# PaddlePaddle/PASSL

Measured on AMD Instinct MI355X. Metric: images/sec/node (2-view), MoCo-v2 R50 bs256/GPU, higher is better.
Workload: dtype bf16; 1 GPU; MoCo-v2 ResNet-50 bf16, bs=256/GPU, 2x224^2 synthetic views, queue=65536, dim=128, T=0.2, m=0.999, momentum-SGD (BASELINE configs[1]); global_batch=256, parallelism=dp1, allocator_retries=0

## Files before the change

include/passl_hip.h:

```cpp
#ifndef PASSL_HIP_H_
#define PASSL_HIP_H_

#include <stdint.h>

#ifdef __cplusplus
extern "C" {
#endif

typedef void* passl_stream_t;

enum passl_status {
  PASSL_OK = 0,
  PASSL_EINVAL = -1,
  PASSL_ELAUNCH = -2,
  PASSL_EUNSUPPORTED = -3
};

enum passl_dtype { PASSL_F32 = 0, PASSL_BF16 = 1 };

#define PASSL_HIP_ABI_VERSION 16
int passl_hip_abi_version(void);
int passl_hip_set_option(const char* name, int value);
int passl_hip_get_option(const char* name, int* value);
int passl_hip_last_igemm_kernel(void);
// ... 105 lines not shown
  int64_t a_sn, a_sh, a_sw;
  int64_t dy_ld;
  float* ws;
  int64_t ws_floats;
  int32_t dtype;
  int32_t splits;
} passl_wgrad_desc;

int passl_hip_slab_reduce(const float* ws, float* out, int64_t n, int slabs, int accumulate,
                          passl_stream_t stream);
int passl_hip_conv_wgrad(const passl_wgrad_desc* d, passl_stream_t stream);


int64_t passl_hip_bn_partial_floats(int nblocks, int C, int shifted);
int passl_hip_bn_stats(const void* x, float* partial, int64_t M, int C, int nblocks, int dtype,
                       passl_stream_t stream);
int passl_hip_bn_finalize(const float* partial, int nblocks, int64_t M, int C, int rows_per_block,
                          const float* gamma, const float* beta, float* running_mean, float* running_var,
                          float momentum, float eps, float* mean, float* invstd, float* scale,
                          float* shift, passl_stream_t stream);
int passl_hip_bn_apply(const void* x, const float* scale, const float* shift, const void* residual,
                       void* z, uint8_t* relu_mask, int64_t M, int C, int relu, int dtype,
                       passl_stream_t stream);
int passl_hip_bn_bwd_reduce(const void* dz, const void* z, const void* x, const float* mean,
                            const float* invstd, const float* scale, const float* shift,
                            float* partial, int64_t M, int C, int nblocks, int relu, int dtype,
                            passl_stream_t stream);
int passl_hip_bn_bwd_finalize(const float* partial, int nblocks, int64_t M, int C,
                              const float* gamma, const float* mean, const float* invstd,
                              float* dgamma, float* dbeta, float* coef ,
                              passl_stream_t stream);
int passl_hip_bn_moments(const float* partial, int nblocks, int64_t M, int C, int rows_per_block, double* mom,
                         passl_stream_t stream);
int passl_hip_bn_finalize_moments(const double* mom_all, int world, int C, const float* gamma, const float* beta,
                                  float* running_mean, float* running_var, float momentum, float eps, float* mean,
                                  float* invstd, float* scale, float* shift, passl_stream_t stream);
int passl_hip_bn_bwd_sums(const float* partial, int nblocks, int64_t M, int C, double* sums, passl_stream_t stream);
int passl_hip_bn_bwd_finalize_sums(const double* sums_all, int world, int rank, int64_t M_total, int C,
                                   const float* gamma, const float* mean, const float* invstd, float* dgamma,
                                   float* dbeta, float* coef, passl_stream_t stream);
int passl_hip_bn_bwd_apply(const void* dz, const void* z, const void* x, const float* coef,
                           const float* scale, const float* shift, void* dx, void* dres, int64_t M,
                           int C, int relu, int dtype, passl_stream_t stream);

int passl_hip_maxpool3x3s2_fwd(const void* x, void* y, uint8_t* idx, int N, int H, int W, int C,
                               int dtype, passl_stream_t stream);
// ... 223 lines not shown
```

passl_amd/csrc/bn.hip:

```cpp
#include <mutex>
#include "common.h"
#include "bn_chunk.h"
#include "options.h"

namespace {

constexpr int kThreads = 256;


template <typename T>
__device__ __forceinline__ void apply_relu_mask(float (&g)[8], const float (&xv)[8], int relu,
                                                const void* zsrc, int64_t chunk,
                                                const float* sc, const float* sh) {
  if (relu == 1) {
    float zz[8];
    ElemTraits<T>::load8(reinterpret_cast<const T*>(zsrc) + chunk * 8, zz);
#pragma unroll
    for (int e = 0; e < 8; ++e) g[e] = zz[e] > 0.f ? g[e] : 0.f;
  } else if (relu == 2) {
#pragma unroll
    for (int e = 0; e < 8; ++e) g[e] = (xv[e] * sc[e] + sh[e]) > 0.f ? g[e] : 0.f;
  } else if (relu == 3) {
    const uint32_t bits = reinterpret_cast<const uint8_t*>(zsrc)[chunk];
#pragma unroll
// ... 342 lines not shown

__global__ void __launch_bounds__(256) bn_bwd_finalize_sums_kernel(
    const double* __restrict__ sums_all, int world, int rank, double m_total, int C,
    const float* __restrict__ gamma, const float* __restrict__ mean, const float* __restrict__ invstd,
    float* __restrict__ dgamma, float* __restrict__ dbeta, float* __restrict__ coef) {
  const int c = blockIdx.x * 256 + threadIdx.x;
  if (c >= C) return;
  double sg = 0.0, sgx = 0.0;
  for (int r = 0; r < world; ++r) {
    sg += sums_all[(int64_t)r * 2 * C + c];
    sgx += sums_all[(int64_t)r * 2 * C + C + c];
  }
  dbeta[c] += (float)sums_all[(int64_t)rank * 2 * C + c];
  dgamma[c] += (float)sums_all[(int64_t)rank * 2 * C + C + c];
  const double gi = (double)gamma[c] * (double)invstd[c];
  const double inv_m = 1.0 / m_total;
  const double B = -gi * (double)invstd[c] * sgx * inv_m;
  const double Cc = -gi * sg * inv_m - B * (double)mean[c];
  coef[c] = (float)gi;
  coef[C + c] = (float)B;
  coef[2 * C + c] = (float)Cc;
}

template <typename T>
__global__ void __launch_bounds__(kThreads) bn_apply_kernel(const T* __restrict__ x,
                                                            const float* __restrict__ scale,
                                                            const float* __restrict__ shift,
                                                            const T* __restrict__ res,
                                                            T* __restrict__ z,
                                                            uint8_t* __restrict__ mask,
                                                            int64_t nchunks, int cols, int relu) {
  const int64_t stride = (int64_t)gridDim.x * kThreads;
  for (int64_t i = (int64_t)blockIdx.x * kThreads + threadIdx.x; i < nchunks; i += stride) {
    const int col = (int)(i % cols);
    float v[8];
    ElemTraits<T>::load8(x + i * 8, v);
    const float4 s0 = *reinterpret_cast<const float4*>(scale + col * 8);
    const float4 s1 = *reinterpret_cast<const float4*>(scale + col * 8 + 4);
    const float4 b0 = *reinterpret_cast<const float4*>(shift + col * 8);
    const float4 b1 = *reinterpret_cast<const float4*>(shift + col * 8 + 4);
    v[0] = v[0] * s0.x + b0.x; v[1] = v[1] * s0.y + b0.y;
    v[2] = v[2] * s0.z + b0.z; v[3] = v[3] * s0.w + b0.w;
    v[4] = v[4] * s1.x + b1.x; v[5] = v[5] * s1.y + b1.y;
    v[6] = v[6] * s1.z + b1.z; v[7] = v[7] * s1.w + b1.w;
    if (res) {
      float r[8];
      ElemTraits<T>::load8(res + i * 8, r);
#pragma unroll
      for (int e = 0; e < 8; ++e) v[e] += r[e];
    }
    if (relu) {
      if (mask) {
        uint32_t bits = 0;
#pragma unroll
        for (int e = 0; e < 8; ++e) bits |= (v[e] > 0.f ? 1u : 0u) << e;
        mask[i] = (uint8_t)bits;
      }
#pragma unroll
      for (int e = 0; e < 8; ++e) v[e] = fmaxf(v[e], 0.f);
    }
    ElemTraits<T>::store8(z + i * 8, v);
  }
}

template <typename T>
__global__ void __launch_bounds__(kThreads) bn_bwd_apply_kernel(
    const T* __restrict__ dz, const void* __restrict__ z, const T* __restrict__ x,
    const float* __restrict__ coef, const float* __restrict__ scale,
    const float* __restrict__ shift, T* __restrict__ dx, T* __restrict__ dres, int64_t nchunks,
    int cols, int C, int relu) {
// ... 2 lines not shown
    const int col = (int)(i % cols);
    float g[8], v[8];
    ElemTraits<T>::load8(dz + i * 8, g);
    ElemTraits<T>::load8(x + i * 8, v);
    if (relu == 2) {
      float sc[8], sh[8];
#pragma unroll
      for (int e = 0; e < 8; ++e) { sc[e] = scale[col * 8 + e]; sh[e] = shift[col * 8 + e]; }
      apply_relu_mask<T>(g, v, 2, nullptr, i, sc, sh);
    } else if (relu) {
      apply_relu_mask<T>(g, v, relu, z, i, nullptr, nullptr);
    }
    float o[8];
#pragma unroll
    for (int e = 0; e < 8; ++e) {
      const int c = col * 8 + e;
      o[e] = coef[c] * g[e] + coef[C + c] * v[e] + coef[2 * C + c];
    }
    ElemTraits<T>::store8(dx + i * 8, o);
    if (dres) ElemTraits<T>::store8(dres + i * 8, g);
  }
}

template <typename T, int U>
__global__ void __launch_bounds__(kThreads) bn_apply_tile_kernel(const T* __restrict__ x,
                                                                 const float* __restrict__ scale,
                                                                 const float* __restrict__ shift,
                                                                 const T* __restrict__ res,
                                                                 T* __restrict__ z,
                                                                 uint8_t* __restrict__ mask,
                                                                 int64_t nchunks, int cols, int relu) {
  const int64_t base = (int64_t)blockIdx.x * (kThreads * U) + threadIdx.x;
  const int col = (int)base & (cols - 1);
  const float4 s0 = *reinterpret_cast<const float4*>(scale + col * 8);
  const float4 s1 = *reinterpret_cast<const float4*>(scale + col * 8 + 4);
  const float4 b0 = *reinterpret_cast<const float4*>(shift + col * 8);
  const float4 b1 = *reinterpret_cast<const float4*>(shift + col * 8 + 4);
  const float sc[8] = {s0.x, s0.y, s0.z, s0.w, s1.x, s1.y, s1.z, s1.w};
  const float sh[8] = {b0.x, b0.y, b0.z, b0.w, b1.x, b1.y, b1.z, b1.w};
  float v[U][8], r[U][8];
#pragma unroll
  for (int u = 0; u < U; ++u) {
    const int64_t i = base + u * kThreads;
    ElemTraits<T>::load8(x + (i < nchunks ? i : nchunks - 1) * 8, v[u]);
  }
  if (res) {
#pragma unroll
    for (int u = 0; u < U; ++u) {
      const int64_t i = base + u * kThreads;
      ElemTraits<T>::load8(res + (i < nchunks ? i : nchunks - 1) * 8, r[u]);
    }
  }
#pragma unroll
  for (int u = 0; u < U; ++u) {
    const int64_t i = base + u * kThreads;
    if (i >= nchunks) break;
    bnc::affine8(v[u], sc, sh);
    if (res) {
#pragma unroll
      for (int e = 0; e < 8; ++e) v[u][e] += r[u][e];
    }
    if (relu) {
      if (mask) {
        uint32_t bits = 0;
#pragma unroll
        for (int e = 0; e < 8; ++e) bits |= (v[u][e] > 0.f ? 1u : 0u) << e;
        mask[i] = (uint8_t)bits;
      }
      bnc::relu8(v[u]);
    }
    ElemTraits<T>::store8(z + i * 8, v[u]);
  }
}

template <typename T, int U>
__global__ void __launch_bounds__(kThreads) bn_bwd_apply_tile_kernel(
    const T* __restrict__ dz, const void* __restrict__ z, const T* __restrict__ x,
    const float* __restrict__ coef, const float* __restrict__ scale,
    const float* __restrict__ shift, T* __restrict__ dx, T* __restrict__ dres, int64_t nchunks,
    int cols, int C, int relu) {
  const int64_t base = (int64_t)blockIdx.x * (kThreads * U) + threadIdx.x;
// ... 95 lines not shown

extern "C" int passl_hip_bn_finalize(const float* partial, int nblocks, int64_t M, int C,
                                     int rows_per_block, const float* gamma, const float* beta,
                                     float* running_mean,
                                     float* running_var, float momentum, float eps, float* mean,
                                     float* invstd, float* scale, float* shift,
                                     passl_stream_t stream) {
  if (!partial || !gamma || !beta || !mean || !invstd || !scale || !shift || M <= 0 || C <= 0 ||
      (C & 7) || nblocks <= 0 || rows_per_block <= 0 || (int64_t)nblocks * rows_per_block < M ||
      (running_mean && !running_var) || !aligned16(partial))
    return PASSL_EINVAL;
  int seg_rows = 0;
  const int nseg = fin_segments(nblocks, true, &seg_rows);
  double* scratch = reinterpret_cast<double*>(const_cast<float*>(partial) + (int64_t)nblocks * C * 3);
  int* counters = nseg > 1 ? fin_counters(C / kFinCh) : nullptr;
  if (nseg > 1 && !counters) return PASSL_ELAUNCH;
  hipLaunchKernelGGL(bn_finalize_kernel, dim3(C / kFinCh, nseg), dim3(kFinThreads), 0, as_stream(stream),
                     partial, nblocks, M, C, rows_per_block, seg_rows, scratch, counters, gamma, beta, running_mean,
                     running_var, momentum, eps, mean, invstd, scale, shift);
  PASSL_RETURN_IF_LAUNCH_FAILED();
  return PASSL_OK;
}

extern "C" int passl_hip_bn_apply(const void* x, const float* scale, const float* shift,
                                  const void* residual, void* z, uint8_t* relu_mask, int64_t M,
                                  int C, int relu, int dtype, passl_stream_t stream) {
  if (!x || !scale || !shift || !z || M <= 0 || C <= 0 || (C & 7) || !aligned16(x) ||
      !aligned16(z) || (residual && !aligned16(residual)) || !aligned16(scale) || !aligned16(shift))
    return PASSL_EINVAL;
  if (relu_mask && !relu) return PASSL_EINVAL;
  const int64_t nchunks = M * (C >> 3);
  const int U = (kThreads % (C >> 3)) == 0 ? passl_opt(Opt::bn_stream_unroll) : 0;
#define PASSL_BN_APPLY_TILE(UU)                                                                          \
  PASSL_DISPATCH_DTYPE(dtype, hipLaunchKernelGGL((bn_apply_tile_kernel<T, UU>),                         \
                                                 dim3((unsigned)((nchunks + kThreads * UU - 1) / (kThreads * UU))), \
                                                 dim3(kThreads), 0, as_stream(stream),                  \
                                                 reinterpret_cast<const T*>(x), scale, shift,           \
                                                 reinterpret_cast<const T*>(residual),                  \
                                                 reinterpret_cast<T*>(z), relu_mask, nchunks, C >> 3, relu);)
  if (U == 2) { PASSL_BN_APPLY_TILE(2) }
  else if (U == 4) { PASSL_BN_APPLY_TILE(4) }
  else if (U == 8) { PASSL_BN_APPLY_TILE(8) }
  else {
    PASSL_DISPATCH_DTYPE(dtype, hipLaunchKernelGGL(bn_apply_kernel<T>, dim3(grid_for(nchunks)),
                                                   dim3(kThreads), 0, as_stream(stream),
                                                   reinterpret_cast<const T*>(x), scale, shift,
                                                   reinterpret_cast<const T*>(residual),
                                                   reinterpret_cast<T*>(z), relu_mask, nchunks, C >> 3,
                                                   relu);)
  }
#undef PASSL_BN_APPLY_TILE
  PASSL_RETURN_IF_LAUNCH_FAILED();
  return PASSL_OK;
}

static bool relu_args_ok(int relu, const void* z, const float* scale, const float* shift) {
  if (relu < 0 || relu > 3) return false;
  if (relu == 1 && (!z || !aligned16(z))) return false;
  if (relu == 2 && (!scale || !shift)) return false;
  if (relu == 3 && !z) return false;
  return true;
}

extern "C" int passl_hip_bn_bwd_reduce(const void* dz, const void* z, const void* x,
                                       const float* mean, const float* invstd,
                                       const float* scale, const float* shift, float* partial,
                                       int64_t M, int C, int nblocks, int relu, int dtype,
                                       passl_stream_t stream) {
  if (!dz || !x || !mean || !invstd || !partial || !relu_args_ok(relu, z, scale, shift) ||
      M <= 0 || C <= 0 || (C & 7) || nblocks <= 0 || !aligned16(dz) || !aligned16(x))
    return PASSL_EINVAL;
  const int rows = (int)((M + nblocks - 1) / nblocks);
  PASSL_DISPATCH_DTYPE(dtype, hipLaunchKernelGGL((bn_reduce_kernel<T, 1>), dim3(nblocks), dim3(kThreads),
                                                 kThreads * 16 * sizeof(float), as_stream(stream),
                                                 reinterpret_cast<const T*>(x),
                                                 reinterpret_cast<const T*>(dz), z, mean, invstd, scale,
// ... 113 lines not shown
```

passl_amd/csrc/bn_chunk.h:

```cpp
#pragma once
#include "common.h"

namespace bnc {

__device__ __forceinline__ void affine8(float (&v)[8], const float (&sc)[8], const float (&sh)[8]) {
#pragma unroll
  for (int e = 0; e < 8; ++e) v[e] = v[e] * sc[e] + sh[e];
}

__device__ __forceinline__ void relu8(float (&v)[8]) {
#pragma unroll
  for (int e = 0; e < 8; ++e) v[e] = fmaxf(v[e], 0.f);
}

__device__ __forceinline__ void bwd8(float (&o)[8], const float (&g)[8], const float (&v)[8], const float (&cA)[8],
                                     const float (&cB)[8], const float (&cC)[8]) {
#pragma unroll
  for (int e = 0; e < 8; ++e) o[e] = __fmaf_rn(cA[e], g[e], cB[e] * v[e]) + cC[e];
}

}
```

passl_amd/hip/config.py:

```python
import os

import torch

_state = {'device': None, 'dtype': torch.bfloat16,
          'fused_bn_stats': os.environ.get('PASSL_FUSED_BN_STATS', '1') != '0',
          'fuse_residual_grad': os.environ.get('PASSL_FUSE_RESIDUAL_GRAD', '1') != '0',
          'fused_bn_backward': os.environ.get('PASSL_FUSED_BN_BACKWARD', '1') != '0',
          'fused_bn_backward2': os.environ.get('PASSL_FUSED_BN_BACKWARD2', '1') != '0',
          'overlap': os.environ.get('PASSL_OVERLAP', '1') != '0',
          'fork_downsample': os.environ.get('PASSL_FORK_DOWNSAMPLE', '1') != '0',
          'side_reductions': os.environ.get('PASSL_SIDE_REDUCTIONS', '1') != '0',
          'fused_stem_pool': os.environ.get('PASSL_FUSED_STEM_POOL', '1') != '0',
          'stem_wgrad_parts': max(1, int(os.environ.get('PASSL_STEM_WGRAD_PARTS', '2') or 1)),
          'stem_tail_flush': os.environ.get('PASSL_STEM_TAIL_FLUSH', '1') != '0',
          'stem_wgrad_main_last': os.environ.get('PASSL_STEM_WGRAD_MAIN_LAST', '1') != '0',
          'side_urgent_rows': int(os.environ.get('PASSL_SIDE_URGENT_ROWS', '500000') or 0),
          'wgrad_halo': int(os.environ.get('PASSL_WGRAD_HALO', '2') or 0),
          'igemm_a_bn': int(os.environ.get('PASSL_IGEMM_A_BN', '0') or 0) & 7,
          'igemm_a_bnb': int(os.environ.get('PASSL_IGEMM_A_BNB', '7') or 0) & 7}


def set_device(name):
    if isinstance(name, torch.device):
        _state['device'] = name
    elif name in ('gpu', 'cuda'):
        _state['device'] = torch.device('cuda', int(os.environ.get('PASSL_DEVICE_INDEX',
                                                                  os.environ.get('LOCAL_RANK', 0))))
        torch.cuda.set_device(_state['device'])
        _cap_memory(_state['device'])
    elif name == 'cpu':
        _state['device'] = torch.device('cpu')
    else:
        raise ValueError("device must be 'gpu' or 'cpu', got %r" % (name,))
    return _state['device']


_capped = set()


def _cap_memory(device):
    if not torch.cuda.is_available() or device.index in _capped:
        return
# ... 61 lines not shown
    return _state['stem_wgrad_main_last']


def side_urgent_rows():
    return _state['side_urgent_rows']


def stem_tail_flush():
    return _state['stem_tail_flush']


def wgrad_halo():
    return _state['wgrad_halo']


def igemm_a_bn(channels):
    return bool(_state['igemm_a_bn'] & _ktile_bit(channels))


def igemm_a_bnb(channels):
    return bool(_state['igemm_a_bnb'] & _ktile_bit(channels))


def _ktile_bit(channels):
    nk = (channels + 63) // 64
    return 1 if nk == 1 else (2 if nk == 2 else 4)


_BOOL_FLAGS = ('fused_bn_stats', 'fuse_residual_grad', 'fused_bn_backward', 'overlap', 'fork_downsample',
               'side_reductions', 'fused_stem_pool', 'fused_bn_backward2', 'stem_tail_flush', 'stem_wgrad_main_last')
_INT_FLAGS = ('stem_wgrad_parts', 'side_urgent_rows', 'wgrad_halo', 'igemm_a_bn', 'igemm_a_bnb')


def set_flag(name, value):
    if name in _BOOL_FLAGS:
        _state[name] = bool(value)
    elif name in _INT_FLAGS:
        _state[name] = max(1, int(value)) if name == 'stem_wgrad_parts' else int(value)
        if name == 'wgrad_halo':
            from . import lib as L
            if L.loaded():
                L.check(L.load().passl_hip_set_option(b'wgrad_halo', int(value)), 'set_option wgrad_halo')
    else:
        raise KeyError('unknown flag %r (known: %s)' % (name, ', '.join(_BOOL_FLAGS + _INT_FLAGS)))


def mirror_library_option(name, value):
    if name == 'wgrad_halo':
        _state['wgrad_halo'] = int(value)
```

passl_amd/hip/lib.py:

```python
import ctypes as C
import os

import torch

_HERE = os.path.dirname(os.path.abspath(__file__))
LIB_PATH = os.path.join(os.path.dirname(_HERE), 'lib', 'libpassl_hip.so')

F32, BF16 = 0, 1
ABI_VERSION = 16
GRAD_CLIP_CHUNK = 16384
_DT = {torch.float32: F32, torch.bfloat16: BF16}

c_p = C.c_void_p
c_i = C.c_int
c_l = C.c_int64
c_f = C.c_float


class ConvDesc(C.Structure):
    _fields_ = [('a', c_p), ('b', c_p), ('y', c_p), ('scale', c_p), ('shift', c_p),
                ('residual', c_p), ('stats', c_p),
                ('bnb_y', c_p), ('bnb_mask', c_p), ('bnb_mean', c_p), ('bnb_invstd', c_p),
                ('bnb_scale', c_p), ('bnb_shift', c_p), ('bnb_partial', c_p),
                ('N', C.c_int32), ('OP', C.c_int32), ('OQ', C.c_int32), ('NCOLS', C.c_int32),
# ... 33 lines not shown

SIGNATURES = {
    'passl_hip_abi_version': (c_i, []),
    'passl_hip_strerror': (C.c_char_p, [c_i]),
    'passl_hip_set_option': (c_i, [C.c_char_p, c_i]),
    'passl_hip_get_option': (c_i, [C.c_char_p, C.POINTER(c_i)]),
    'passl_hip_last_igemm_kernel': (c_i, []),
    'passl_hip_ema_update': (c_i, [c_p, c_p, c_p, c_l, c_f, c_p]),
    'passl_hip_bn_fold': (c_i, [c_p, c_p, c_p, c_p, c_p, c_l, c_f, c_p, c_p, c_p]),
    'passl_hip_momentum_sgd': (c_i, [c_p, c_p, c_p, c_l, c_f, c_f, c_f, c_f, c_p]),
    'passl_hip_momentum_sgd_dev': (c_i, [c_p, c_p, c_p, c_l, c_p, c_f, c_f, c_f, c_p]),
    'passl_hip_cast_f32_to_bf16': (c_i, [c_p, c_p, c_l, c_p]),
    'passl_hip_pack_weights': (c_i, [c_p, c_p, c_i, c_p, c_p, c_p, c_i, c_p]),
    'passl_hip_nchw_to_nhwc_pad': (c_i, [c_p, c_p, c_i, c_i, c_i, c_i, c_i, c_i, c_i, c_i, c_p]),
    'passl_hip_conv_igemm': (c_i, [C.POINTER(ConvDesc), c_p]),
    'passl_hip_conv_igemm_apro': (c_i, [C.POINTER(ConvDesc), C.POINTER(ConvApro), c_p]),
    'passl_hip_conv_wgrad': (c_i, [C.POINTER(WgradDesc), c_p]),
    'passl_hip_slab_reduce': (c_i, [c_p, c_p, c_l, c_i, c_i, c_p]),
    'passl_hip_bn_partial_floats': (c_l, [c_i, c_i, c_i]),
    'passl_hip_bn_stats': (c_i, [c_p, c_p, c_l, c_i, c_i, c_i, c_p]),
    'passl_hip_bn_finalize': (c_i, [c_p, c_i, c_l, c_i, c_i, c_p, c_p, c_p, c_p, c_f, c_f, c_p, c_p,
                                    c_p, c_p, c_p]),
    'passl_hip_bn_apply': (c_i, [c_p, c_p, c_p, c_p, c_p, c_p, c_l, c_i, c_i, c_i, c_p]),
    'passl_hip_bn_bwd_reduce': (c_i, [c_p, c_p, c_p, c_p, c_p, c_p, c_p, c_p, c_l, c_i, c_i, c_i,
                                      c_i, c_p]),
    'passl_hip_bn_bwd_finalize': (c_i, [c_p, c_i, c_l, c_i, c_p, c_p, c_p, c_p, c_p, c_p, c_p]),
    'passl_hip_bn_moments': (c_i, [c_p, c_i, c_l, c_i, c_i, c_p, c_p]),
    'passl_hip_bn_finalize_moments': (c_i, [c_p, c_i, c_i, c_p, c_p, c_p, c_p, c_f, c_f, c_p, c_p, c_p, c_p, c_p]),
    'passl_hip_bn_bwd_sums': (c_i, [c_p, c_i, c_l, c_i, c_p, c_p]),
    'passl_hip_bn_bwd_finalize_sums': (c_i, [c_p, c_i, c_i, c_l, c_i, c_p, c_p, c_p, c_p, c_p, c_p, c_p]),
    'passl_hip_bn_bwd_apply': (c_i, [c_p, c_p, c_p, c_p, c_p, c_p, c_p, c_p, c_l, c_i, c_i, c_i,
                                     c_p]),
    'passl_hip_maxpool3x3s2_fwd': (c_i, [c_p, c_p, c_p, c_i, c_i, c_i, c_i, c_i, c_p]),
    'passl_hip_maxpool3x3s2_bwd': (c_i, [c_p, c_p, c_p, c_i, c_i, c_i, c_i, c_i, c_p]),
    'passl_hip_bn_relu_maxpool_blocks': (c_i, [c_i, c_i, c_i, c_i]),
    'passl_hip_bn_relu_maxpool_fwd': (c_i, [c_p, c_p, c_p, c_p, c_p, c_i, c_i, c_i, c_i, c_i, c_p]),
    'passl_hip_bn_relu_maxpool_bwd_reduce': (c_i, [c_p, c_p, c_p, c_p, c_p, c_p, c_p, c_p, c_i, c_i, c_i, c_i, c_i, c_i,
                                                   c_p]),
    'passl_hip_bn_relu_maxpool_bwd_apply': (c_i, [c_p, c_p, c_p, c_p, c_p, c_p, c_p, c_i, c_i, c_i, c_i, c_i, c_p]),
    'passl_hip_avgpool_fwd': (c_i, [c_p, c_p, c_i, c_i, c_i, c_i, c_p]),
    'passl_hip_avgpool_bwd': (c_i, [c_p, c_p, c_i, c_i, c_i, c_i, c_p]),
    'passl_hip_relu_bwd': (c_i, [c_p, c_p, c_p, c_l, c_i, c_p]),
    'passl_hip_colsum': (c_i, [c_p, c_p, c_l, c_i, c_i, c_p, c_l, c_p]),
    'passl_hip_colsum_acc': (c_i, [c_p, c_p, c_l, c_i, c_i, c_p, c_l, c_p]),
    'passl_hip_l2norm_fwd': (c_i, [c_p, c_p, c_p, c_i, c_i, c_f, c_p]),
    'passl_hip_l2norm_bwd': (c_i, [c_p, c_p, c_p, c_p, c_i, c_i, c_i, c_p]),
# ... 182 lines not shown
```

passl_amd/hip/nn.py:

```python
from types import SimpleNamespace

import torch
import torch.nn as tnn
from torch.autograd import Function

from . import config, ops, streams
from . import plan as P
from .packer import WeightPacker


class Layer(tnn.Module):

    def sublayers(self, include_self=False):
        mods = list(self.modules())
        return mods if include_self else mods[1:]

    def set_state_dict(self, sd, *a, **k):
        return self.load_state_dict(sd, *a, **k)


def _need_rt(layer):
    if getattr(layer, '_rt', None) is None:
        raise RuntimeError('%s is not attached to an EncoderArena (call EncoderArena(encoder) after '
                           'building the model)' % type(layer).__name__)
# ... 299 lines not shown
        y = torch.empty(N, pl.fd.OP, pl.fd.OQ, self.geom.cout, dtype=x.dtype, device=x.device)
        scale = shift = None
        if bn is not None:
            scale, shift = bn.infer_affine()
        ops.conv_igemm(pl.fd, x, rt.w_fwd, y, scale=scale, shift=shift, residual=residual, relu=relu)
        return y


def _collectives_active():
    from ..core.sync_utils import collectives_active
    return collectives_active()


def convert_sync_batchnorm(module):
    for m in module.modules():
        if isinstance(m, _BatchNormBase):
            m._sync = True
    return module


class _BNActFn(Function):
    @staticmethod
    def forward(ctx, y, gamma, beta, residual, layer, relu, partial, res_slot, link_box, res_link=None, pend_box=None,
                dylink=None):
        has_res = residual is not None
        ctx.sync = bool(getattr(layer, '_sync', False)) and _collectives_active()
        z, st, mask = ops.bn_train_fwd(y, gamma.detach(), beta.detach(), layer._mean,
                                       layer._variance, residual, relu, layer._momentum,
                                       layer._epsilon, partial=partial,
                                       want_mask=relu and has_res, sync=ctx.sync, apply=pend_box is None)
        if pend_box is not None:
            z = torch.empty_like(y)
            pend_box[0] = BNPending(y, st[2], st[3])
        ctx.relu_mode = 0 if not relu else (3 if has_res else 2)
        if layer._rt is not None and any(ctx.needs_input_grad):
            layer._rt.arena.expect_grad(layer._rt.indices)
        ctx.save_for_backward(y, st, mask)
        ctx.layer, ctx.has_res, ctx.res_slot = layer, has_res, res_slot
        ctx.link = None
        ctx.dylink = dylink
        if link_box is not None:
            ctx.link = link_box[0] = BNLink(y, st, mask, ctx.relu_mode,
                                            res_link if (has_res and ctx.relu_mode == 3 and res_slot is None) else None)
        return z

    @staticmethod
    def backward(ctx, dz):
        y, st, mask = ctx.saved_tensors
        layer = ctx.layer
        streams.autograd_node_entry(dz.device)
        if layer.affine:
            for p in (layer.weight, layer.bias):
                if p.grad is None:
                    p.grad = ops.zeros_like(p)
            gamma, dgamma, dbeta = layer.weight.detach(), layer.weight.grad, layer.bias.grad
        else:
            gamma, dgamma, dbeta = layer._const[0], layer._dscratch[0], layer._dscratch[1]
        want_dres = ctx.has_res and (ctx.needs_input_grad[3] or ctx.res_slot is not None)
        fused = ctx.link.fused if ctx.link is not None else None
        if ctx.link is not None:
            ctx.link.y = ctx.link.st = ctx.link.mask = ctx.link.fused = ctx.link.res_link = None
        if fused is not None and fused[0].is_cuda:
            fused[0].record_stream(torch.cuda.current_stream(dz.device))
        dz = dz.contiguous()
        defer = (fused is not None and ctx.dylink is not None and ctx.needs_input_grad[0] and
                 dz.dtype == torch.bfloat16)
        out = ops.bn_bwd(dz, mask, y, gamma, st[0], st[1], dgamma, dbeta, relu=ctx.relu_mode,
                         want_dres=want_dres, scale=st[2], shift=st[3], fused=fused, sync=ctx.sync, defer=defer)
        dx, dres = out[0], out[1]
        if defer:
            ctx.dylink.put(dz, y, out[2], dx)
        if ctx.res_slot is not None:
            ctx.res_slot.put(dres)
            dres = None
        if layer._rt is not None:
            layer._rt.arena.grad_ready(layer._rt.indices)
        return dx, None, None, dres, None, None, None, None, None, None, None, None


class _BatchNormBase(Layer):

    def __init__(self, num_features, momentum=0.9, epsilon=1e-05, weight_attr=None,
                 bias_attr=None, data_format='NCHW', use_global_stats=None, name=None):
        super().__init__()
        dev = config.get_device()
        self._momentum, self._epsilon = momentum, epsilon
        self._use_global_stats = use_global_stats
        self.num_features = num_features
        if (weight_attr is False) != (bias_attr is False):
            raise NotImplementedError('BatchNorm with only one of weight / bias')
        self.affine = weight_attr is not False
        if self.affine:
            self.weight = tnn.Parameter(torch.ones(num_features, device=dev))
            self.bias = tnn.Parameter(torch.zeros(num_features, device=dev))
        else:
            self.weight = self.bias = None
            self.register_buffer('_const', torch.stack([torch.ones(num_features, device=dev),
                                                        torch.zeros(num_features, device=dev)]), persistent=False)
            self.register_buffer('_dscratch', torch.zeros(2, num_features, device=dev), persistent=False)
        self.register_buffer('_mean', torch.zeros(num_features, device=dev))
# ... 5 lines not shown
            else (not self.training)

    def infer_affine(self):
        rt = self._rt
        if rt is not None and rt.arena.bn_affine is not None:
            s, e = rt.bn_slice
            return rt.arena.bn_affine[0][s:e], rt.arena.bn_affine[1][s:e]
        gamma, beta = self.gamma_beta()
        scale = gamma * torch.rsqrt(self._variance + self._epsilon)
        return scale, beta - self._mean * scale

    def gamma_beta(self):
        if self.affine:
            return self.weight.detach(), self.bias.detach()
        return self._const[0], self._const[1]

    def forward(self, y, residual=None, relu=False, stats=None, res_slot=None, res_link=None, consumer=None,
                sole_reader=False):
        if self.uses_global_stats():
            if torch.is_grad_enabled() and (y.requires_grad or (self.affine and self.weight.requires_grad)):
                raise NotImplementedError('frozen BatchNorm inside a differentiated graph is not on '
                                          'the MoCo hot path (key encoder runs under no_grad)')
            scale, shift = self.infer_affine()
            return ops.bn_apply(y, scale, shift, residual, relu)
        box = [None] if (torch.is_grad_enabled() and y.dtype == torch.bfloat16 and
                         config.fused_bn_backward()) else None
        gamma, beta = (self.weight, self.bias) if self.affine else (self._const[0], self._const[1])
        pend = [None] if (consumer is not None and _apply_in_consumer(consumer, y, residual, relu, stats)) else None
        z = _BNActFn.apply(y, gamma, beta, residual, self, relu, stats, res_slot, box, res_link, pend,
                           dy_link(y) if sole_reader else None)
        if box is not None and box[0] is not None:
            z._passl_bn_link = box[0]
        if pend is not None:
            z._passl_bn_pending = pend[0]
        return z


class BatchNorm2D(_BatchNormBase):
    pass


class BatchNorm1D(_BatchNormBase):
    pass


class _MaxPoolFn(Function):
    @staticmethod
    def forward(ctx, x):
        y, idx = ops.maxpool_fwd(x)
        ctx.save_for_backward(idx)
        ctx.hw = (x.shape[1], x.shape[2])
        return y

# ... 657 lines not shown
```

passl_amd/hip/ops.py:

```python
import ctypes as C
import math

import torch

from . import config
from . import lib as L
from . import plan as P


def _lib():
    return L.load()


class _Workspace:

    def __init__(self):
        self._bufs = {}

    def get(self, n_floats, device):
        key = (device.type, device.index, L.stream() if device.type == 'cuda' else 0)
        buf = self._bufs.get(key)
        if buf is None or buf.numel() < n_floats:
            buf = torch.empty(max(int(n_floats), 1 << 20), dtype=torch.float32, device=device)
            self._bufs[key] = buf
# ... 201 lines not shown
def _bn_blocks(M, Cch, cap=1024):
    lanes = max(1, 256 // max(Cch // 8, 1))
    return int(max(1, min(cap, -(-M // (16 * lanes)))))


def conv_stats_buffer(d: P.Desc, device):
    t = conv_tiles(d)
    return torch.empty(bn_partial_floats(t, d.NCOLS, True), dtype=torch.float32, device=device), t


def bn_partial_floats(nblocks, Cch, shifted):
    return nblocks * Cch * (3 if shifted else 2) + 16 * Cch * 4


def _gather_doubles(t):
    import torch.distributed as dist
    world = dist.get_world_size()
    out = torch.empty((world * t.shape[0],) + tuple(t.shape[1:]), dtype=t.dtype, device=t.device)
    dist.all_gather_into_tensor(out, t)
    return out.view((world,) + tuple(t.shape))


def bn_train_fwd(x, gamma, beta, rmean, rvar, residual=None, relu=True, momentum=0.9, eps=1e-5,
                 partial=None, want_mask=False, sync=False, apply=True):
    Cch = x.shape[-1]
    M = x.numel() // Cch
    dev = x.device
    stats = torch.empty(4, Cch, dtype=torch.float32, device=dev)
    lib, st, dtc = _lib(), L.stream(), L.dt(x)
    if partial is None:
        nb = _bn_blocks(M, Cch)
        rpb = -(-M // nb)
        nb = -(-M // rpb)
        partial = torch.empty(bn_partial_floats(nb, Cch, True), dtype=torch.float32, device=dev)
        L.check(lib.passl_hip_bn_stats(L.ptr(x), L.ptr(partial), M, Cch, nb, dtc, st), 'bn_stats')
    else:
        partial, nb = partial
        rpb = 128
    if sync:
        mom = torch.empty(3, Cch, dtype=torch.float64, device=dev)
        L.check(lib.passl_hip_bn_moments(L.ptr(partial), nb, M, Cch, rpb, L.ptr(mom), st), 'bn_moments')
        mom_all = _gather_doubles(mom)
        L.check(lib.passl_hip_bn_finalize_moments(L.ptr(mom_all), mom_all.shape[0], Cch, L.ptr(gamma), L.ptr(beta),
                                                  L.ptr(rmean), L.ptr(rvar), momentum, eps, L.ptr(stats[0]),
                                                  L.ptr(stats[1]), L.ptr(stats[2]), L.ptr(stats[3]), L.stream()),
                'bn_finalize_moments')
    else:
        L.check(lib.passl_hip_bn_finalize(L.ptr(partial), nb, M, Cch, rpb, L.ptr(gamma), L.ptr(beta),
                                          L.ptr(rmean), L.ptr(rvar), momentum, eps,
                                          L.ptr(stats[0]), L.ptr(stats[1]), L.ptr(stats[2]),
                                          L.ptr(stats[3]), st), 'bn_finalize')
    if not apply:
        return None, stats, None
    z = torch.empty_like(x)
    mask = torch.empty(x.numel() // 8, dtype=torch.uint8, device=dev) if (want_mask and relu) \
        else None
    L.check(lib.passl_hip_bn_apply(L.ptr(x), L.ptr(stats[2]), L.ptr(stats[3]), L.ptr(residual),
                                   L.ptr(z), L.ptr(mask), M, Cch, 1 if relu else 0, dtc, L.stream()),
            'bn_apply')
    return z, stats, mask


def bn_apply(x, scale, shift, residual=None, relu=False, out=None):
    Cch = x.shape[-1]
    M = x.numel() // Cch
    z = torch.empty_like(x) if out is None else out
    L.check(_lib().passl_hip_bn_apply(L.ptr(x), L.ptr(scale), L.ptr(shift), L.ptr(residual),
                                      L.ptr(z), None, M, Cch, 1 if relu else 0, L.dt(x),
                                      L.stream()), 'bn_apply')
    return z


def bn_bwd(dz, z, x, gamma, mean, invstd, dgamma, dbeta, relu=True, want_dres=False,
           scale=None, shift=None, fused=None, sync=False, defer=False):
    Cch = x.shape[-1]
    M = x.numel() // Cch
    dev = x.device
    coef = torch.empty(3 * Cch, dtype=torch.float32, device=dev)
    lib, st, dtc = _lib(), L.stream(), L.dt(x)
    r = int(relu)
    zp = L.ptr(z) if r in (1, 3) else None
    if fused is not None:
        partial, nb = fused
        r, zp = 0, None
    else:
        nb = _bn_blocks(M, Cch, cap=768)
        partial = torch.empty(bn_partial_floats(nb, Cch, False), dtype=torch.float32, device=dev)
        L.check(lib.passl_hip_bn_bwd_reduce(L.ptr(dz), zp, L.ptr(x), L.ptr(mean), L.ptr(invstd),
                                            L.ptr(scale), L.ptr(shift), L.ptr(partial), M, Cch, nb, r,
                                            dtc, st), 'bn_bwd_reduce')
    if sync:
        import torch.distributed as dist
# ... 886 lines not shown
```

passl_amd/modeling/backbones/resnet.py:

```python
import torch

from ...hip import config, nn, ops, plan as P, streams
from ...modules import init
from ...utils.logger import get_logger
from ...modules.freeze import freeze_batchnorm_statictis
from .builder import BACKBONES


class BottleneckBlock(nn.Layer):
    expansion = 4

    def __init__(self, inplanes, planes, stride=1, downsample=None, groups=1, base_width=64,
                 dilation=1, norm_layer=None):
        super().__init__()
        norm_layer = norm_layer or nn.BatchNorm2D
        width = int(planes * (base_width / 64.)) * groups
        self.conv1 = nn.Conv2D(inplanes, width, 1, bias_attr=False)
        self.bn1 = norm_layer(width)
        self.conv2 = nn.Conv2D(width, width, 3, padding=dilation, stride=stride, groups=groups,
                               dilation=dilation, bias_attr=False)
        self.bn2 = norm_layer(width)
        self.conv3 = nn.Conv2D(width, planes * self.expansion, 1, bias_attr=False)
        self.bn3 = norm_layer(planes * self.expansion)
        self.relu = nn.ReLU()
# ... 1 lines not shown
        self.stride = stride

    def forward(self, x):
        slot = None
        if config.fuse_residual_grad() and torch.is_grad_enabled() and x.requires_grad:
            slot = nn.GradSlot()
            slot.arm()
        fork = (self.downsample is not None and torch.is_grad_enabled() and x.requires_grad and
                streams.enabled(x) and config.fork_downsample() and not torch.cuda.is_current_stream_capturing())
        x_ready = streams.record_event(torch.cuda.current_stream(x.device)) if fork else None
        out, st = self.conv1(x, want_stats=True, add_slot=slot,
                             producer=nn.bn_link(x) if slot is not None else None)
        out = self.bn1(out, relu=True, stats=st, sole_reader=True)
        out, st = self.conv2(out, want_stats=True, producer=nn.bn_link(out))
        out = self.bn2(out, relu=True, stats=st, consumer=self.conv3)
        out, st3 = self.conv3(out, want_stats=True, producer=nn.bn_link(out), pending=nn.bn_pending(out))
        if self.downsample is not None:
            if fork:
                main = torch.cuda.current_stream(x.device)
                side = streams.fork_stream(x.device)
                streams.wait_event(side, x_ready)
                with torch.cuda.stream(side):
                    idn, st = self.downsample[0](x, want_stats=True, sink_slot=slot)
                    identity = self.downsample[1](idn, relu=False, stats=st, sole_reader=True)
                streams.wait_event(main, streams.record_event(side))
            else:
                idn, st = self.downsample[0](x, want_stats=True, sink_slot=slot)
                identity = self.downsample[1](idn, relu=False, stats=st, sole_reader=True)
            return self.bn3(out, residual=identity, relu=True, stats=st3, res_link=nn.bn_link(identity),
                            sole_reader=True)
        return self.bn3(out, residual=x, relu=True, stats=st3, res_slot=slot, sole_reader=True)

    def forward_frozen(self, x, allow_fork=True):
        fork = allow_fork and self.downsample is not None and streams.enabled(x) and config.fork_downsample()
        x_ready = streams.record_event(torch.cuda.current_stream(x.device)) if fork else None
        out = self.conv1.infer(x, self.bn1, relu=True)
        out = self.conv2.infer(out, self.bn2, relu=True)
        identity = x
        if fork:
            main, side = torch.cuda.current_stream(x.device), streams.fork_stream(x.device)
            streams.wait_event(side, x_ready)
            with torch.cuda.stream(side):
                identity = self.downsample[0].infer(x, self.downsample[1], relu=False)
            streams.wait_event(main, streams.record_event(side))
        elif self.downsample is not None:
            identity = self.downsample[0].infer(x, self.downsample[1], relu=False)
        return self.conv3.infer(out, self.bn3, residual=identity, relu=True)


class BasicBlock(nn.Layer):
    expansion = 1
# ... 3 lines not shown
        super().__init__()
        norm_layer = norm_layer or nn.BatchNorm2D
        if dilation > 1:
            raise NotImplementedError('Dilation > 1 not supported in BasicBlock')
        self.conv1 = nn.Conv2D(inplanes, planes, 3, stride=stride, padding=1, bias_attr=False)
        self.bn1 = norm_layer(planes)
        self.relu = nn.ReLU()
        self.conv2 = nn.Conv2D(planes, planes, 3, padding=1, bias_attr=False)
        self.bn2 = norm_layer(planes)
        self.downsample = downsample
        self.stride = stride

    def forward(self, x):
        slot = None
        if (config.fuse_residual_grad() and torch.is_grad_enabled() and x.requires_grad and self.stride == 1):
            slot = nn.GradSlot()
            slot.arm()
        out, st = self.conv1(x, want_stats=True, add_slot=slot,
                             producer=nn.bn_link(x) if slot is not None else None)
        out = self.bn1(out, relu=True, stats=st)
        out, st2 = self.conv2(out, want_stats=True, producer=nn.bn_link(out))
        if self.downsample is not None:
            idn, st = self.downsample[0](x, want_stats=True, sink_slot=slot)
            identity = self.downsample[1](idn, relu=False, stats=st)
            return self.bn2(out, residual=identity, relu=True, stats=st2)
        return self.bn2(out, residual=x, relu=True, stats=st2, res_slot=slot)

    def forward_frozen(self, x, allow_fork=True):
        out = self.conv1.infer(x, self.bn1, relu=True)
        identity = x if self.downsample is None else self.downsample[0].infer(x, self.downsample[1], relu=False)
        return self.conv2.infer(out, self.bn2, residual=identity, relu=True)


class _StagedInput:
    __slots__ = ('xp', 'H', 'W', 'ready')

    def __init__(self, xp, H, W, ready):
        self.xp, self.H, self.W, self.ready = xp, H, W, ready


@BACKBONES.register()
class ResNet(nn.Layer):
    stem_pool = True

    def __init__(self, depth, num_classes=0, with_pool=False, zero_init_residual=False,
                 frozen_stages=-1, pretrained=None):
        super().__init__()
# ... 161 lines not shown
```

Before: 11410 images/sec.

## Fuse downsample BN apply into the block's final BN residual-add kernel

The downsample branch's BatchNorm no longer writes its normalized output. It leaves a pending (y, scale, shift) record, and the block's final BN apply kernel normalizes the residual on the fly, with bf16 rounding to match the old numerics. A new bn_apply2 entry point and a templated ResAffine path in both apply kernels support this. This removes one full elementwise read-write pass and one kernel launch per downsample block, at the cost of extra per-channel loads in the final apply and more complex pending-state plumbing through autograd.

```diff
diff --git a/include/passl_hip.h b/include/passl_hip.h
--- a/include/passl_hip.h
+++ b/include/passl_hip.h
@@ -151,6 +151,9 @@
 int passl_hip_bn_apply(const void* x, const float* scale, const float* shift, const void* residual,
                        void* z, uint8_t* relu_mask, int64_t M, int C, int relu, int dtype,
                        passl_stream_t stream);
+int passl_hip_bn_apply2(const void* x, const float* scale, const float* shift, const void* res,
+                        const float* res_scale, const float* res_shift, void* z, uint8_t* relu_mask,
+                        int64_t M, int C, int relu, int dtype, passl_stream_t stream);
 int passl_hip_bn_bwd_reduce(const void* dz, const void* z, const void* x, const float* mean,
                             const float* invstd, const float* scale, const float* shift,
                             float* partial, int64_t M, int C, int nblocks, int relu, int dtype,
diff --git a/passl_amd/csrc/bn.hip b/passl_amd/csrc/bn.hip
--- a/passl_amd/csrc/bn.hip
+++ b/passl_amd/csrc/bn.hip
@@ -388,14 +388,17 @@
   coef[2 * C + c] = (float)Cc;
 }
 
-template <typename T>
+struct ResAffine { const float* scale; const float* shift; };
+
+template <typename T, typename... R>
 __global__ void __launch_bounds__(kThreads) bn_apply_kernel(const T* __restrict__ x,
                                                             const float* __restrict__ scale,
                                                             const float* __restrict__ shift,
                                                             const T* __restrict__ res,
                                                             T* __restrict__ z,
                                                             uint8_t* __restrict__ mask,
-                                                            int64_t nchunks, int cols, int relu) {
+                                                            int64_t nchunks, int cols, int relu, const R... ra_) {
+  constexpr bool RA = sizeof...(R) != 0;
   const int64_t stride = (int64_t)gridDim.x * kThreads;
   for (int64_t i = (int64_t)blockIdx.x * kThreads + threadIdx.x; i < nchunks; i += stride) {
     const int col = (int)(i % cols);
@@ -409,9 +412,21 @@
     v[2] = v[2] * s0.z + b0.z; v[3] = v[3] * s0.w + b0.w;
     v[4] = v[4] * s1.x + b1.x; v[5] = v[5] * s1.y + b1.y;
     v[6] = v[6] * s1.z + b1.z; v[7] = v[7] * s1.w + b1.w;
-    if (res) {
+    if (RA || res) {
       float r[8];
       ElemTraits<T>::load8(res + i * 8, r);
+      if constexpr (RA) {
+        const ResAffine& ra = (ra_, ...);
+        const float4 rs0 = *reinterpret_cast<const float4*>(ra.scale + col * 8);
+        const float4 rs1 = *reinterpret_cast<const float4*>(ra.scale + col * 8 + 4);
+        const float4 rb0 = *reinterpret_cast<const float4*>(ra.shift + col * 8);
+        const float4 rb1 = *reinterpret_cast<const float4*>(ra.shift + col * 8 + 4);
+        r[0] = r[0] * rs0.x + rb0.x; r[1] = r[1] * rs0.y + rb0.y;
+        r[2] = r[2] * rs0.z + rb0.z; r[3] = r[3] * rs0.w + rb0.w;
+        r[4] = r[4] * rs1.x + rb1.x; r[5] = r[5] * rs1.y + rb1.y;
+        r[6] = r[6] * rs1.z + rb1.z; r[7] = r[7] * rs1.w + rb1.w;
+        bnc::round8<T>(r);
+      }
 #pragma unroll
       for (int e = 0; e < 8; ++e) v[e] += r[e];
     }
@@ -460,14 +475,15 @@
   }
 }
 
-template <typename T, int U>
+template <typename T, int U, typename... R>
 __global__ void __launch_bounds__(kThreads) bn_apply_tile_kernel(const T* __restrict__ x,
                                                                  const float* __restrict__ scale,
                                                                  const float* __restrict__ shift,
                                                                  const T* __restrict__ res,
                                                                  T* __restrict__ z,
                                                                  uint8_t* __restrict__ mask,
-                                                                 int64_t nchunks, int cols, int relu) {
+                                                                 int64_t nchunks, int cols, int relu, const R... ra_) {
+  constexpr bool RA = sizeof...(R) != 0;
   const int64_t base = (int64_t)blockIdx.x * (kThreads * U) + threadIdx.x;
   const int col = (int)base & (cols - 1);
   const float4 s0 = *reinterpret_cast<const float4*>(scale + col * 8);
@@ -476,13 +492,23 @@
   const float4 b1 = *reinterpret_cast<const float4*>(shift + col * 8 + 4);
   const float sc[8] = {s0.x, s0.y, s0.z, s0.w, s1.x, s1.y, s1.z, s1.w};
   const float sh[8] = {b0.x, b0.y, b0.z, b0.w, b1.x, b1.y, b1.z, b1.w};
+  float rsc[8], rsh[8];
+  if constexpr (RA) {
+    const ResAffine& ra = (ra_, ...);
+    const float4 rs0 = *reinterpret_cast<const float4*>(ra.scale + col * 8);
+    const float4 rs1 = *reinterpret_cast<const float4*>(ra.scale + col * 8 + 4);
+    const float4 rb0 = *reinterpret_cast<const float4*>(ra.shift + col * 8);
+    const float4 rb1 = *reinterpret_cast<const float4*>(ra.shift + col * 8 + 4);
+    rsc[0] = rs0.x; rsc[1] = rs0.y; rsc[2] = rs0.z; rsc[3] = rs0.w; rsc[4] = rs1.x; rsc[5] = rs1.y; rsc[6] = rs1.z; rsc[7] = rs1.w;
+    rsh[0] = rb0.x; rsh[1] = rb0.y; rsh[2] = rb0.z; rsh[3] = rb0.w; rsh[4] = rb1.x; rsh[5] = rb1.y; rsh[6] = rb1.z; rsh[7] = rb1.w;
+  }
   float v[U][8], r[U][8];
 #pragma unroll
   for (int u = 0; u < U; ++u) {
     const int64_t i = base + u * kThreads;
     ElemTraits<T>::load8(x + (i < nchunks ? i : nchunks - 1) * 8, v[u]);
   }
-  if (res) {
+  if (RA || res) {
 #pragma unroll
     for (int u = 0; u < U; ++u) {
       const int64_t i = base + u * kThreads;
@@ -493,8 +519,12 @@
   for (int u = 0; u < U; ++u) {
     const int64_t i = base + u * kThreads;
     if (i >= nchunks) break;
+    if (RA) {
+      bnc::affine8(r[u], rsc, rsh);
+      bnc::round8<T>(r[u]);
+    }
     bnc::affine8(v[u], sc, sh);
-    if (res) {
+    if (RA || res) {
 #pragma unroll
       for (int e = 0; e < 8; ++e) v[u][e] += r[u][e];
     }
@@ -636,36 +666,61 @@
   return PASSL_OK;
 }
 
-extern "C" int passl_hip_bn_apply(const void* x, const float* scale, const float* shift,
-                                  const void* residual, void* z, uint8_t* relu_mask, int64_t M,
-                                  int C, int relu, int dtype, passl_stream_t stream) {
+template <bool RA>
+static int bn_apply_launch(const void* x, const float* scale, const float* shift, const void* residual,
+                           const float* res_scale, const float* res_shift, void* z, uint8_t* relu_mask, int64_t M,
+                           int C, int relu, int dtype, passl_stream_t stream) {
   if (!x || !scale || !shift || !z || M <= 0 || C <= 0 || (C & 7) || !aligned16(x) ||
       !aligned16(z) || (residual && !aligned16(residual)) || !aligned16(scale) || !aligned16(shift))
+    return PASSL_EINVAL;
+  if (RA && (!residual || !res_scale || !res_shift || !aligned16(res_scale) || !aligned16(res_shift)))
     return PASSL_EINVAL;
   if (relu_mask && !relu) return PASSL_EINVAL;
   const int64_t nchunks = M * (C >> 3);
   const int U = (kThreads % (C >> 3)) == 0 ? passl_opt(Opt::bn_stream_unroll) : 0;
+  const ResAffine ra = {res_scale, res_shift};
+#define PASSL_BN_APPLY_ARGS                                                                              \
+  reinterpret_cast<const T*>(x), scale, shift, reinterpret_cast<const T*>(residual), reinterpret_cast<T*>(z), relu_mask, \
+      nchunks, C >> 3, relu
 #define PASSL_BN_APPLY_TILE(UU)                                                                          \
-  PASSL_DISPATCH_DTYPE(dtype, hipLaunchKernelGGL((bn_apply_tile_kernel<T, UU>),                         \
-                                                 dim3((unsigned)((nchunks + kThreads * UU - 1) / (kThreads * UU))), \
-                                                 dim3(kThreads), 0, as_stream(stream),                  \
-                                                 reinterpret_cast<const T*>(x), scale, shift,           \
-                                                 reinterpret_cast<const T*>(residual),                  \
-                                                 reinterpret_cast<T*>(z), relu_mask, nchunks, C >> 3, relu);)
+  PASSL_DISPATCH_DTYPE(dtype, {                                                                          \
+    const dim3 grid((unsigned)((nchunks + kThreads * UU - 1) / (kThreads * UU)));                        \
+    if constexpr (RA)                                                                                    \
+      hipLaunchKernelGGL((bn_apply_tile_kernel<T, UU, ResAffine>), grid, dim3(kThreads), 0, as_stream(stream), \
+                         PASSL_BN_APPLY_ARGS, ra);                                                       \
+    else                                                                                                 \
+      hipLaunchKernelGGL((bn_apply_tile_kernel<T, UU>), grid, dim3(kThreads), 0, as_stream(stream),      \
+                         PASSL_BN_APPLY_ARGS);                                                           \
+  })
   if (U == 2) { PASSL_BN_APPLY_TILE(2) }
   else if (U == 4) { PASSL_BN_APPLY_TILE(4) }
   else if (U == 8) { PASSL_BN_APPLY_TILE(8) }
   else {
-    PASSL_DISPATCH_DTYPE(dtype, hipLaunchKernelGGL(bn_apply_kernel<T>, dim3(grid_for(nchunks)),
-                                                   dim3(kThreads), 0, as_stream(stream),
-                                                   reinterpret_cast<const T*>(x), scale, shift,
-                                                   reinterpret_cast<const T*>(residual),
-                                                   reinterpret_cast<T*>(z), relu_mask, nchunks, C >> 3,
-                                                   relu);)
-  }
+    PASSL_DISPATCH_DTYPE(dtype, {
+      if constexpr (RA)
+        hipLaunchKernelGGL((bn_apply_kernel<T, ResAffine>), dim3(grid_for(nchunks)), dim3(kThreads), 0,
+                           as_stream(stream), PASSL_BN_APPLY_ARGS, ra);
+      else
+        hipLaunchKernelGGL(bn_apply_kernel<T>, dim3(grid_for(nchunks)), dim3(kThreads), 0, as_stream(stream),
+                           PASSL_BN_APPLY_ARGS);
+    })
+  }
+#undef PASSL_BN_APPLY_ARGS
 #undef PASSL_BN_APPLY_TILE
   PASSL_RETURN_IF_LAUNCH_FAILED();
   return PASSL_OK;
+}
+
+extern "C" int passl_hip_bn_apply(const void* x, const float* scale, const float* shift,
+                                  const void* residual, void* z, uint8_t* relu_mask, int64_t M,
+                                  int C, int relu, int dtype, passl_stream_t stream) {
+  return bn_apply_launch<false>(x, scale, shift, residual, nullptr, nullptr, z, relu_mask, M, C, relu, dtype, stream);
+}
+
+extern "C" int passl_hip_bn_apply2(const void* x, const float* scale, const float* shift, const void* res,
+                                   const float* res_scale, const float* res_shift, void* z, uint8_t* relu_mask,
+                                   int64_t M, int C, int relu, int dtype, passl_stream_t stream) {
+  return bn_apply_launch<true>(x, scale, shift, res, res_scale, res_shift, z, relu_mask, M, C, relu, dtype, stream);
 }
 
 static bool relu_args_ok(int relu, const void* z, const float* scale, const float* shift) {
diff --git a/passl_amd/csrc/bn_chunk.h b/passl_amd/csrc/bn_chunk.h
--- a/passl_amd/csrc/bn_chunk.h
+++ b/passl_amd/csrc/bn_chunk.h
@@ -13,6 +13,18 @@
   for (int e = 0; e < 8; ++e) v[e] = fmaxf(v[e], 0.f);
 }
 
+template <typename T>
+__device__ __forceinline__ void round8(float (&v)[8]) {
+  if constexpr (sizeof(T) == 2) {
+#pragma unroll
+    for (int e = 0; e < 8; e += 2) {
+      const uint32_t u = pack2bf(v[e], v[e + 1]);
+      v[e] = __uint_as_float(u << 16);
+      v[e + 1] = __uint_as_float(u & 0xffff0000u);
+    }
+  }
+}
+
 __device__ __forceinline__ void bwd8(float (&o)[8], const float (&g)[8], const float (&v)[8], const float (&cA)[8],
                                      const float (&cB)[8], const float (&cC)[8]) {
 #pragma unroll
diff --git a/passl_amd/hip/config.py b/passl_amd/hip/config.py
--- a/passl_amd/hip/config.py
+++ b/passl_amd/hip/config.py
@@ -17,7 +17,8 @@
           'side_urgent_rows': int(os.environ.get('PASSL_SIDE_URGENT_ROWS', '500000') or 0),
           'wgrad_halo': int(os.environ.get('PASSL_WGRAD_HALO', '2') or 0),
           'igemm_a_bn': int(os.environ.get('PASSL_IGEMM_A_BN', '0') or 0) & 7,
-          'igemm_a_bnb': int(os.environ.get('PASSL_IGEMM_A_BNB', '7') or 0) & 7}
+          'igemm_a_bnb': int(os.environ.get('PASSL_IGEMM_A_BNB', '7') or 0) & 7,
+          'bn_dual_apply': os.environ.get('PASSL_BN_DUAL_APPLY', '1') != '0'}
 
 
 def set_device(name):
@@ -125,13 +126,18 @@
     return bool(_state['igemm_a_bnb'] & _ktile_bit(channels))
 
 
+def bn_dual_apply():
+    return _state['bn_dual_apply']
+
+
 def _ktile_bit(channels):
     nk = (channels + 63) // 64
     return 1 if nk == 1 else (2 if nk == 2 else 4)
 
 
 _BOOL_FLAGS = ('fused_bn_stats', 'fuse_residual_grad', 'fused_bn_backward', 'overlap', 'fork_downsample',
-               'side_reductions', 'fused_stem_pool', 'fused_bn_backward2', 'stem_tail_flush', 'stem_wgrad_main_last')
+               'side_reductions', 'fused_stem_pool', 'fused_bn_backward2', 'stem_tail_flush', 'stem_wgrad_main_last',
+               'bn_dual_apply')
 _INT_FLAGS = ('stem_wgrad_parts', 'side_urgent_rows', 'wgrad_halo', 'igemm_a_bn', 'igemm_a_bnb')
 
 
diff --git a/passl_amd/hip/lib.py b/passl_amd/hip/lib.py
--- a/passl_amd/hip/lib.py
+++ b/passl_amd/hip/lib.py
@@ -79,6 +79,7 @@
     'passl_hip_bn_finalize': (c_i, [c_p, c_i, c_l, c_i, c_i, c_p, c_p, c_p, c_p, c_f, c_f, c_p, c_p,
                                     c_p, c_p, c_p]),
     'passl_hip_bn_apply': (c_i, [c_p, c_p, c_p, c_p, c_p, c_p, c_l, c_i, c_i, c_i, c_p]),
+    'passl_hip_bn_apply2': (c_i, [c_p, c_p, c_p, c_p, c_p, c_p, c_p, c_p, c_l, c_i, c_i, c_i, c_p]),
     'passl_hip_bn_bwd_reduce': (c_i, [c_p, c_p, c_p, c_p, c_p, c_p, c_p, c_p, c_l, c_i, c_i, c_i,
                                       c_i, c_p]),
     'passl_hip_bn_bwd_finalize': (c_i, [c_p, c_i, c_l, c_i, c_p, c_p, c_p, c_p, c_p, c_p, c_p]),
diff --git a/passl_amd/hip/nn.py b/passl_amd/hip/nn.py
--- a/passl_amd/hip/nn.py
+++ b/passl_amd/hip/nn.py
@@ -345,13 +345,14 @@
 class _BNActFn(Function):
     @staticmethod
     def forward(ctx, y, gamma, beta, residual, layer, relu, partial, res_slot, link_box, res_link=None, pend_box=None,
-                dylink=None):
+                dylink=None, res_pending=None):
         has_res = residual is not None
         ctx.sync = bool(getattr(layer, '_sync', False)) and _collectives_active()
         z, st, mask = ops.bn_train_fwd(y, gamma.detach(), beta.detach(), layer._mean,
-                                       layer._variance, residual, relu, layer._momentum,
-                                       layer._epsilon, partial=partial,
-                                       want_mask=relu and has_res, sync=ctx.sync, apply=pend_box is None)
+                                       layer._variance, residual if res_pending is None else res_pending.y, relu,
+                                       layer._momentum, layer._epsilon, partial=partial,
+                                       want_mask=relu and has_res, sync=ctx.sync, apply=pend_box is None,
+                                       res_affine=None if res_pending is None else (res_pending.scale, res_pending.shift))
         if pend_box is not None:
             z = torch.empty_like(y)
             pend_box[0] = BNPending(y, st[2], st[3])
@@ -398,7 +399,7 @@
             dres = None
         if layer._rt is not None:
             layer._rt.arena.grad_ready(layer._rt.indices)
-        return dx, None, None, dres, None, None, None, None, None, None, None, None
+        return dx, None, None, dres, None, None, None, None, None, None, None, None, None
 
 
 class _BatchNormBase(Layer):
@@ -450,13 +451,19 @@
                 raise NotImplementedError('frozen BatchNorm inside a differentiated graph is not on '
                                           'the MoCo hot path (key encoder runs under no_grad)')
             scale, shift = self.infer_affine()
+            rp = bn_pending(residual) if residual is not None else None
+            if rp is not None:
+                return ops.bn_apply(y, scale, shift, rp.y, relu, res_affine=(rp.scale, rp.shift))
             return ops.bn_apply(y, scale, shift, residual, relu)
         box = [None] if (torch.is_grad_enabled() and y.dtype == torch.bfloat16 and
                          config.fused_bn_backward()) else None
         gamma, beta = (self.weight, self.bias) if self.affine else (self._const[0], self._const[1])
-        pend = [None] if (consumer is not None and _apply_in_consumer(consumer, y, residual, relu, stats)) else None
+        if isinstance(consumer, _BatchNormBase):
+            pend = [None] if (not relu and residual is None and config.bn_dual_apply()) else None
+        else:
+            pend = [None] if (consumer is not None and _apply_in_consumer(consumer, y, residual, relu, stats)) else None
         z = _BNActFn.apply(y, gamma, beta, residual, self, relu, stats, res_slot, box, res_link, pend,
-                           dy_link(y) if sole_reader else None)
+                           dy_link(y) if sole_reader else None, bn_pending(residual) if residual is not None else None)
         if box is not None and box[0] is not None:
             z._passl_bn_link = box[0]
         if pend is not None:
diff --git a/passl_amd/hip/ops.py b/passl_amd/hip/ops.py
--- a/passl_amd/hip/ops.py
+++ b/passl_amd/hip/ops.py
@@ -247,7 +247,7 @@
 
 
 def bn_train_fwd(x, gamma, beta, rmean, rvar, residual=None, relu=True, momentum=0.9, eps=1e-5,
-                 partial=None, want_mask=False, sync=False, apply=True):
+                 partial=None, want_mask=False, sync=False, apply=True, res_affine=None):
     Cch = x.shape[-1]
     M = x.numel() // Cch
     dev = x.device
@@ -280,19 +280,27 @@
     z = torch.empty_like(x)
     mask = torch.empty(x.numel() // 8, dtype=torch.uint8, device=dev) if (want_mask and relu) \
         else None
-    L.check(lib.passl_hip_bn_apply(L.ptr(x), L.ptr(stats[2]), L.ptr(stats[3]), L.ptr(residual),
-                                   L.ptr(z), L.ptr(mask), M, Cch, 1 if relu else 0, dtc, L.stream()),
-            'bn_apply')
+    _bn_apply_launch(x, stats[2], stats[3], residual, res_affine, z, mask, M, Cch, relu)
     return z, stats, mask
 
 
-def bn_apply(x, scale, shift, residual=None, relu=False, out=None):
+def _bn_apply_launch(x, scale, shift, residual, res_affine, z, mask, M, Cch, relu):
+    if res_affine is None:
+        L.check(_lib().passl_hip_bn_apply(L.ptr(x), L.ptr(scale), L.ptr(shift), L.ptr(residual), L.ptr(z), L.ptr(mask),
+                                          M, Cch, 1 if relu else 0, L.dt(x), L.stream()), 'bn_apply')
+        return
+    if residual is None or residual.shape != x.shape or residual.dtype != x.dtype:
+        raise ValueError('bn_apply: a residual affine needs a residual of the shape and dtype of x')
+    L.check(_lib().passl_hip_bn_apply2(L.ptr(x), L.ptr(scale), L.ptr(shift), L.ptr(residual), L.ptr(res_affine[0]),
+                                       L.ptr(res_affine[1]), L.ptr(z), L.ptr(mask), M, Cch, 1 if relu else 0,
+                                       L.dt(x), L.stream()), 'bn_apply2')
+
+
+def bn_apply(x, scale, shift, residual=None, relu=False, out=None, res_affine=None, mask=None):
     Cch = x.shape[-1]
     M = x.numel() // Cch
     z = torch.empty_like(x) if out is None else out
-    L.check(_lib().passl_hip_bn_apply(L.ptr(x), L.ptr(scale), L.ptr(shift), L.ptr(residual),
-                                      L.ptr(z), None, M, Cch, 1 if relu else 0, L.dt(x),
-                                      L.stream()), 'bn_apply')
+    _bn_apply_launch(x, scale, shift, residual, res_affine, z, mask, M, Cch, relu)
     return z
 
 
diff --git a/passl_amd/modeling/backbones/resnet.py b/passl_amd/modeling/backbones/resnet.py
--- a/passl_amd/modeling/backbones/resnet.py
+++ b/passl_amd/modeling/backbones/resnet.py
@@ -47,11 +47,11 @@
                 streams.wait_event(side, x_ready)
                 with torch.cuda.stream(side):
                     idn, st = self.downsample[0](x, want_stats=True, sink_slot=slot)
-                    identity = self.downsample[1](idn, relu=False, stats=st, sole_reader=True)
+                    identity = self.downsample[1](idn, relu=False, stats=st, sole_reader=True, consumer=self.bn3)
                 streams.wait_event(main, streams.record_event(side))
             else:
                 idn, st = self.downsample[0](x, want_stats=True, sink_slot=slot)
-                identity = self.downsample[1](idn, relu=False, stats=st, sole_reader=True)
+                identity = self.downsample[1](idn, relu=False, stats=st, sole_reader=True, consumer=self.bn3)
             return self.bn3(out, residual=identity, relu=True, stats=st3, res_link=nn.bn_link(identity),
                             sole_reader=True)
         return self.bn3(out, residual=x, relu=True, stats=st3, res_slot=slot, sole_reader=True)
@@ -101,7 +101,7 @@
         out, st2 = self.conv2(out, want_stats=True, producer=nn.bn_link(out))
         if self.downsample is not None:
             idn, st = self.downsample[0](x, want_stats=True, sink_slot=slot)
-            identity = self.downsample[1](idn, relu=False, stats=st)
+            identity = self.downsample[1](idn, relu=False, stats=st, consumer=self.bn2)
             return self.bn2(out, residual=identity, relu=True, stats=st2)
         return self.bn2(out, residual=x, relu=True, stats=st2, res_slot=slot)
 
```

Result: no change. 11460 images/sec, median of 6 (+0.5%).
